# HUSRCF/JaTSR-Just-audio-transformer-super-solution

Measured on AMD Instinct MI355X. Metric: DiT latent-frames/sec (B=28,C=1024,T=512, 50-step CFG), higher is better.
Workload: dtype bf16; 1 GPU; v3mod2 DiT 50-step CFG=3.0 flow-matching sampling, hipGraph, B=28/GPU C=1024 T=512; B_per_gpu=28, global_batch=28, T=512, C=1024, euler_steps=50, weights=recipe (random-init, non-zero adaLN/final), parallelism=replicas x1, no collective in the loop, rccl_ranks=1

## Files before the change

jatsr-just-audio-transformer-super-solution_amd/csrc/elementwise.hip:

```cpp
#include "jat_kernels.h"
#include "jat_gelu.h"
#include "jat_dtype.h"
#include <cstdlib>

__device__ __forceinline__ unsigned short f2bf_e(float f) { return jat_f2op(f); }
__device__ __forceinline__ uint2 pack4_e(float a, float b, float c, float d) {
  uint2 r;
  r.x = jat_pack2(a, b);
  r.y = jat_pack2(c, d);
  return r;
}
__device__ __forceinline__ float wave_sum(float v) {
#pragma unroll
  for (int o = 32; o > 0; o >>= 1) v += __shfl_xor(v, o);
  return v;
}
__device__ __forceinline__ float silu_f(float x) { return x / (1.0f + __expf(-x)); }

__global__ void __launch_bounds__(256) norm_modulate_kernel(const float* __restrict__ x, const float* __restrict__ w,
                                                            const float* __restrict__ shift,
                                                            const float* __restrict__ scale, int64_t mod_bstride,
                                                            bf16_t* __restrict__ y, int M, int D, int ntok, int mode) {
  const int lane = threadIdx.x & 63;
  const int row = blockIdx.x * 4 + (threadIdx.x >> 6);
// ... 184 lines not shown
      const uint2 v = *(const uint2*)(tile + r * ROW + part * 8);
      *(uint2*)(A + ((int64_t)b * ntok + tok0 + r) * Ktot + (int64_t)c0 * 4 + part * 4) = v;
    }
  }
}

hipError_t launch_patchify(const float* x_t, const float* x_cond, bf16_t* A, int B, int B_src, int cond_zero_from,
                           int C_t, int C_c, int T_orig, int ntok, hipStream_t s, const int* tvalid) {
  if (C_t % 32 != 0 || C_c % 32 != 0 || B <= 0 || B_src <= 0) return hipErrorInvalidValue;
  dim3 grid((ntok + 63) / 64, (C_t + C_c) / 32, B);
  hipLaunchKernelGGL(patchify_kernel, grid, dim3(256), 0, s, x_t, x_cond, A, B_src, cond_zero_from, C_t, C_c, T_orig,
                     ntok, tvalid);
  return hipGetLastError();
}

__global__ void time_sinusoid_kernel(const float* __restrict__ t, float* __restrict__ e, int B, int D) {
  const int half = D >> 1;
  const int i = blockIdx.x * blockDim.x + threadIdx.x;
  if (i >= B * half) return;
  const int b = i / half, k = i - b * half;
  const float c = logf(10000.0f) / (float)(half - 1);
  const float f = expf((float)k * -c);
  const float a = t[b] * f;
  e[(int64_t)b * D + k] = sinf(a);
  e[(int64_t)b * D + half + k] = cosf(a);
}
hipError_t launch_time_sinusoid(const float* t, float* e, int B, int D, hipStream_t s) {
  const int n = B * (D / 2);
  hipLaunchKernelGGL(time_sinusoid_kernel, dim3((n + 255) / 256), dim3(256), 0, s, t, e, B, D);
  return hipGetLastError();
// ... 392 lines not shown
```

jatsr-just-audio-transformer-super-solution_amd/csrc/gemm.hip:

```cpp
#include "jat_kernels.h"
#include "jat_dtype.h"

#include <type_traits>

typedef jat_opx8 bf16x8;
typedef __attribute__((ext_vector_type(4))) float f32x4;
typedef __attribute__((ext_vector_type(4))) unsigned u32x4;
typedef __attribute__((address_space(3))) void* lds_ptr_t;

template <int I, int N, class F>
__device__ __forceinline__ void static_for(F&& f) {
  if constexpr (I < N) {
    f(std::integral_constant<int, I>{});
    static_for<I + 1, N>(f);
  }
}

__device__ __forceinline__ unsigned short f2bf(float f) { return jat_f2op(f); }
__device__ __forceinline__ uint2 pack4(float a, float b, float c, float d) {
  uint2 r;
  r.x = jat_pack2(a, b);
  r.y = jat_pack2(c, d);
  return r;
}
#include "jat_gelu.h"
__device__ __forceinline__ uint2 gelu_pack4(float a, float b, float c, float d) {
  f32x2 g[2] = {f32x2{a, b}, f32x2{c, d}};
  gelu_erf_n<2>(g);
  return pack4(g[0][0], g[0][1], g[1][0], g[1][1]);
}

__device__ __forceinline__ float2 rope_rot(float a, float b, float c, float s) {
  return float2{__builtin_fmaf(a, c, -(b * s)), __builtin_fmaf(b, c, a * s)};
}

template <int TM>
__device__ __forceinline__ void rows_rstd_issue(const GemmArgs& p, int row0, int lane, f32x4 (&rsv)[TM]) {
  const int lg = p.rs_np >> 3;
  const int rpi = 64 >> lg;
#pragma unroll
  for (int t = 0; t < TM; ++t) {
    const int row = min(row0 + t * rpi + (lane >> lg), p.M - 1);
    const float* ptr = p.rs_part + (int64_t)row * p.rs_np + (lane & ((1 << lg) - 1)) * 4;
    asm volatile("global_load_dwordx4 %0, %1, off" : "=v"(rsv[t]) : "v"(ptr) : "memory");
  }
}
template <int TM, int YOUNGER>
__device__ __forceinline__ void rows_rstd_reduce(const GemmArgs& p, f32x4 (&rsv)[TM], float (&sums)[TM]) {
  asm volatile("s_waitcnt vmcnt(%0)" ::"n"(YOUNGER) : "memory");
#pragma unroll
  for (int t = 0; t < TM; ++t) asm volatile("" : "+v"(rsv[t]));
  const int lpr = p.rs_np >> 2;
#pragma unroll
  for (int t = 0; t < TM; ++t) {
    float sq = (rsv[t][0] + rsv[t][1]) + (rsv[t][2] + rsv[t][3]);
    if (lpr >= 2) sq += __shfl_xor(sq, 1);
    if (lpr >= 4) sq += __shfl_xor(sq, 2);
// ... 53 lines not shown
  JAT_TL(0) JAT_TLR(5)
#else
#define JAT_TL(i)
#define JAT_TLX(i)
#define JAT_TLR(i)
#define JAT_TL_FLUSH()
#endif
  if (p.ksplit > 1) {
    const int z = blockIdx.y;
    p.A += (int64_t)z * p.K;
    p.W += (int64_t)z * p.K;
    p.out = (float*)p.out + (int64_t)z * p.split_stride;
  }
  constexpr int BM = WM * TM * 16, BN = WN * TN * 16, BK = 64;
  constexpr int NW = WM * WN;
  constexpr int A_BYTES = BM * 128, B_BYTES = BN * 128, STAGE = A_BYTES + B_BYTES;
  constexpr int PA = BM / 8, PB = BN / 8;
  constexpr int AI = (PA + NW - 1) / NW, BI = (PB + NW - 1) / NW;
  static_assert(BM % 8 == 0 && BN % 8 == 0, "tile rows must be a multiple of 8");
  extern __shared__ __attribute__((aligned(16))) char smem[];

  const int tid = threadIdx.x, lane = tid & 63;
  const int wave = __builtin_amdgcn_readfirstlane(tid >> 6);
  const int wm = wave / WN, wn = wave % WN;

  const int tiles_m = (p.M + BM - 1) / BM, tiles_n = p.N / BN;
  int id;
  {
    const int nwg = gridDim.x, bid = blockIdx.x;
    const int q = nwg >> 3, r = nwg & 7, xcd = bid & 7;
    id = (xcd < r ? xcd * (q + 1) : r * (q + 1) + (xcd - r) * q) + (bid >> 3);
  }
  constexpr int GROUP = 8;
  const int per_group = GROUP * tiles_n;
  const int first_m = (id / per_group) * GROUP;
  const int gsz = min(tiles_m - first_m, GROUP);
  const int in_g = id % per_group;
  const int m0 = (first_m + in_g % gsz) * BM;
  const int n0 = (in_g / gsz) * BN;

  const int srow = lane >> 3;
  const int schunk = (lane & 7) ^ srow;
  const bf16_t* a_src[AI];
  const bf16_t* b_src[BI];
#pragma unroll
  for (int j = 0; j < AI; ++j) {
    const int r = min(wave + j * NW, PA - 1) * 8 + srow;
    const int gm = min(m0 + r, p.M - 1);
    a_src[j] = p.A + (int64_t)gm * p.lda + schunk * 8;
  }
#pragma unroll
  for (int j = 0; j < BI; ++j) {
    const int r = min(wave + j * NW, PB - 1) * 8 + srow;
// ... 41 lines not shown
    for (int j = 0; j < TN; ++j) wf[j] = *(const bf16x8*)(sB + b_row_off + j * 2048 + coff);
  };
  auto mma = [&](const bf16x8(&af)[TM], const bf16x8(&wf)[TN]) {
#pragma unroll
    for (int i = 0; i < TM; ++i)
#pragma unroll
      for (int j = 0; j < TN; ++j)
        acc[i][j] = JAT_MFMA_16x16x32(wf[j], af[i], acc[i][j], 0, 0, 0);
  };

  float rstd_rows[TM], rstd_sums[TM];
  [[maybe_unused]] f32x4 rstd_raw[TM];
#pragma unroll
  for (int i = 0; i < TM; ++i) rstd_rows[i] = 1.0f;
  if (p.rs_part) {
    rows_rstd_issue<TM>(p, m0 + wm * TM * 16, lane, rstd_raw);
    if constexpr (PIPE != 8) rows_rstd_reduce<TM, 0>(p, rstd_raw, rstd_sums);
  }

  const int nk = p.K / BK;
  if constexpr (PIPE == 6) {
    static_assert(NW == 8 && PA % 4 == 0 && PB % 4 == 0, "PIPE 6: 8 MFMA waves + 4 DMA waves");
    constexpr int NDW = 4, AI6 = PA / NDW, BI6 = PB / NDW;
    if (wave >= NW) {
      const int dw = wave - NW;
      const bf16_t* asrc[AI6];
      const bf16_t* bsrc[BI6];
#pragma unroll
      for (int j = 0; j < AI6; ++j)
        asrc[j] = p.A + (int64_t)min(m0 + (dw + j * NDW) * 8 + srow, p.M - 1) * p.lda + schunk * 8;
#pragma unroll
// ... 55 lines not shown
      cur = cur == 2 ? 0 : cur + 1;
    }
    if (grp == 0) __builtin_amdgcn_s_barrier();
  } else if constexpr (PIPE == 8) {
    static_assert(NW == 8, "quadrant ping-pong needs two waves per SIMD in one block");
    constexpr bool SPLIT_M = TM * TN > 20;
    constexpr int TMa = SPLIT_M ? (TM + 1) / 2 : TM, TMb = TM - TMa, TNa = (TN + 1) / 2, TNb = TN - TNa;
    constexpr int PA0 = WM * TMa * 2, PA1 = WM * TMb * 2, PB0 = WN * TNa * 2, PB1 = WN * TNb * 2;
    constexpr int CA0 = (PA0 + 7) / 8, CA1 = (PA1 + 7) / 8, CB0 = (PB0 + 7) / 8, CB1 = (PB1 + 7) / 8;
    constexpr int CTILE = CA0 + CA1 + CB0 + CB1;
    const int grp = wave >> 2;
    const char* a_base = (const char*)(p.A + (int64_t)m0 * p.lda);
    const char* b_base = (const char*)(p.W + (int64_t)n0 * p.ldw);
    unsigned oa0[CA0], oa1[CA1 > 0 ? CA1 : 1], ob0[CB0], ob1[CB1];
    int la0[CA0], la1[CA1 > 0 ? CA1 : 1], lb0[CB0], lb1[CB1];
    auto piece_row = [&](int q, int per, int tiles, int first) {
      const int w = q / per, in = q - w * per;
      return w * tiles * 16 + first * 16 + in * 8;
    };
#pragma unroll
    for (int j = 0; j < CA0; ++j) {
      const int r = piece_row(min(wave + 8 * j, PA0 - 1), TMa * 2, TM, 0);
      oa0[j] = (unsigned)((min(m0 + r + srow, p.M - 1) - m0) * (int)p.lda * 2 + schunk * 16);
      la0[j] = r * 128;
    }
#pragma unroll
    for (int j = 0; j < CA1; ++j) {
      const int r = piece_row(min(wave + 8 * j, PA1 - 1), TMb * 2, TM, TMa);
      oa1[j] = (unsigned)((min(m0 + r + srow, p.M - 1) - m0) * (int)p.lda * 2 + schunk * 16);
      la1[j] = r * 128;
    }
    auto piece_row_b = [&](int q, int per, int first) {
      const int w = q / per, in = q - w * per;
      return ctile(w, first + (in >> 1)) * 16 + (in & 1) * 8;
    };
#pragma unroll
    for (int j = 0; j < CB0; ++j) {
      const int r = piece_row_b(min(wave + 8 * j, PB0 - 1), TNa * 2, 0);
      ob0[j] = (unsigned)((r + srow) * (int)p.ldw * 2 + schunk * 16);
      lb0[j] = A_BYTES + r * 128;
    }
#pragma unroll
    for (int j = 0; j < CB1; ++j) {
      const int r = piece_row_b(min(wave + 8 * j, PB1 - 1), TNb * 2, TNa);
// ... 625 lines not shown
        const int d = dt * 16 + frow, ch = kk * 4 + fg;
        const bf16x8 vf = *(const bf16x8*)(smem + SV + d * 256 + (ch >> 3) * 128 + (((ch & 7) ^ (d & 7)) << 4));
#pragma unroll
        for (int h = 0; h < G; ++h) o[h][dt] = JAT_MFMA_16x16x32(vf, pf[h][kk], o[h][dt], 0, 0, 0);
      }
    JAT_TLX(4)
    if (m0 + q < p.M) {
#pragma unroll
      for (int h = 0; h < G; ++h) {
        bf16_t* op = (bf16_t*)p.out + (int64_t)(m0 + q) * p.ldo + (hbase + h) * 64 + fg * 4;
#pragma unroll
        for (int dt = 0; dt < 4; ++dt)
          *(uint2*)(op + dt * 16) = pack4(o[h][dt][0] * inv[h], o[h][dt][1] * inv[h], o[h][dt][2] * inv[h], o[h][dt][3] * inv[h]);
      }
    }
    JAT_TL_FLUSH()
    return;
  }

#pragma unroll
  for (int i = 0; i < TM; ++i) {
    const int m = m0 + wm * TM * 16 + i * 16 + frow;
    if (m >= p.M) continue;
    int b = 0, pos = m;
    if constexpr (EPI == EPI_RESID || EPI == EPI_QKV_ROPE || EPI == EPI_UNPATCH) {
      b = m / p.ntok;
      pos = m - b * p.ntok;
    }
    const float rstd_d = rstd_rows[i];
#pragma unroll
// ... 660 lines not shown
}

template <int WM, int WN, int TM, int TN, int PIPE, int CE, int EPI>
static hipError_t launch_one(const GemmArgs& a, hipStream_t s) {
  constexpr int BM = WM * TM * 16, BN = WN * TN * 16;
  constexpr int LDS = (PIPE == 6 ? 3 : 2) * (BM + BN) * 128;
  static_assert(LDS <= 160 * 1024, "tile does not fit the 160 KiB LDS");
  static bool attr_set = false;
  auto kern = gemm_bf16_kernel<WM, WN, TM, TN, PIPE, CE, EPI>;
  if (!attr_set) {
    hipError_t e = hipFuncSetAttribute((const void*)kern, hipFuncAttributeMaxDynamicSharedMemorySize, LDS);
    if (e != hipSuccess) return e;
    attr_set = true;
  }
  if (a.N % BN != 0 || a.K % 64 != 0 || a.M <= 0) return hipErrorInvalidValue;
  const int tiles = ((a.M + BM - 1) / BM) * (a.N / BN);
  if (a.ksplit > 1 && EPI != EPI_F32) return hipErrorInvalidValue;
  hipLaunchKernelGGL(kern, dim3(tiles, a.ksplit > 1 ? a.ksplit : 1), dim3((WM * WN + (PIPE == 6 ? 4 : 0)) * 64), LDS, s, a);
  return hipGetLastError();
}

template <int WM, int WN, int TM, int TN, int PIPE, int CE = 0>
static hipError_t launch_epi(const GemmArgs& a, int epi, hipStream_t s) {
  switch (epi) {
    case EPI_F32: return launch_one<WM, WN, TM, TN, PIPE, CE, EPI_F32>(a, s);
    case EPI_BF16: return launch_one<WM, WN, TM, TN, PIPE, CE, EPI_BF16>(a, s);
    case EPI_BF16_GELU: return launch_one<WM, WN, TM, TN, PIPE, CE, EPI_BF16_GELU>(a, s);
    case EPI_RESID: return launch_one<WM, WN, TM, TN, PIPE, CE, EPI_RESID>(a, s);
    case EPI_QKV_ROPE: return launch_one<WM, WN, TM, TN, PIPE, CE, EPI_QKV_ROPE>(a, s);
    case EPI_UNPATCH: return launch_one<WM, WN, TM, TN, PIPE, CE, EPI_UNPATCH>(a, s);
  }
// ... 24 lines not shown

hipError_t launch_qkv_attn(const GemmArgs& a, hipStream_t s) {
  if (a.ntok != 128 || a.N % 448 != 0 || a.M % 128 != 0) return hipErrorInvalidValue;
  return launch_one<2, 4, 4, 7, 8, 0, EPI_QKV_ATTN>(a, s);
}
void gemm_variant_tile(int variant, int* bm, int* bn) {
  *bm = kVariantTile[variant][0];
  *bn = kVariantTile[variant][1];
}

bool gemm_variant_exists(int variant) {
  return variant >= 0 && variant < gemm_num_variants() && kVariantTile[variant][0] != 0;
}

hipError_t launch_gemm(const GemmArgs& a, int epi, int variant, hipStream_t s) {
  if (!gemm_variant_exists(variant)) return hipErrorInvalidValue;
  if (a.N % kVariantTile[variant][1] != 0) variant = (a.N % 128 == 0) ? 20 : 10;
  switch (variant) {
    case 10: return launch_epi<2, 2, 4, 2, 1>(a, epi, s);
    case 18: return launch_epi<2, 2, 4, 5, 2, 1>(a, epi, s);
    case 20: return launch_epi<2, 2, 4, 4, 2, 1>(a, epi, s);
    case 21: return launch_epi<2, 4, 8, 4, 2, 1>(a, epi, s);
    case 25: return launch_epi<4, 2, 4, 5, 6, 1>(a, epi, s);
    case 26: return launch_epi<4, 2, 4, 4, 6, 1>(a, epi, s);
    case 27: return launch_epi<2, 2, 2, 5, 2, 1>(a, epi, s);
    case 28: return launch_epi<2, 2, 2, 4, 2, 1>(a, epi, s);
    case 31: return launch_epi<2, 4, 7, 5, 8, 1>(a, epi, s);
    case 39:
      if (gemm_kpair_part_eligible(a, epi)) return launch_kpair<EPI_F32, 0, true>(a, s);
      if (gemm_kpair_eligible(a, epi))
// ... 14 lines not shown
```

jatsr-just-audio-transformer-super-solution_amd/csrc/jat_api.cpp:

```cpp
#include "../../include/jat_hip.h"

#include <hip/hip_runtime.h>

#include <cmath>
#include <cstdarg>
#include <cstdio>
#include <cstdlib>
#include <cstring>
#include <string>
#include <unordered_map>
#include <vector>

#include "jat_internal.h"
#include "jat_dtype.h"

static thread_local char g_err[512] = "";
int jat_fail(int code, const char* fmt, ...) {
  va_list ap;
  va_start(ap, fmt);
  vsnprintf(g_err, sizeof(g_err), fmt, ap);
  va_end(ap);
  return code;
}

// ... 478 lines not shown
      JCHK(gemm(m, G_FC2, w.hm, m->mlp, L.w2, m->mlp, M, D, m->mlp, EPI_F32, p, s));
      if (can_fuse && !f && next) {
        KCHK(launch_splitk_resid_norm(w.kpart, split, (int64_t)M * D, L.b2, mod_l + 5 * D, bstride, w.x, next->w, next->shift,
                                      next->scale, bstride, w.xn, M, D, ntok, m->cfg.norm_mode, s));
        if (next_done) *next_done = true;
      } else {
        KCHK(launch_splitk_resid_finish(w.kpart, split, (int64_t)M * D, L.b2, mod_l + 5 * D, bstride, ntok, w.x, M, D, s));
      }
    } else {
      JCHK(gemm(m, G_FC2, w.hm, m->mlp, L.w2, m->mlp, M, D, m->mlp, EPI_RESID, e, s));
    }
  }
  return JAT_OK;
}

static int forward_impl(const jat_model* m, const Workspace& w, const float* x_t, int B_src, const float* x_cond,
                        int cond_zero_from, const float* t, const float* mod, int64_t mod_bstride, float* x_pred,
                        int B, int T, hipStream_t s, const Fold* f = nullptr, const float* pc = nullptr) {
  const int ntok = (T + 3) / 4, M = B * ntok, D = m->D;
  if (!mod) {
    JCHK(time_path(m, w, t, B, s));
    JCHK(adaln_path(m, w.t_silu, w.mod, B, 0, m->depth, s));
    mod = w.mod;
    mod_bstride = (int64_t)m->depth * 6 * D;
  }
  if (t) HIPCHK(hipMemsetAsync(w.vt, 0, w.vt_bytes, s));
  auto patch_split = [&](int rows, int K) {
    if (!m->sw.patch_split || m->variants[G_OTHER] >= 0 || m->bott % 128 != 0) return 1;
    const int tiles = ((rows + 63) / 64) * (m->bott / 128);
    if (tiles > 128 && K < 8192) return 1;
    int split = 512 / tiles, cap = m->mlp / (2 * m->bott);
    if (cap > 4) cap = 4;
    if (split > cap) split = cap;
    while (split > 1 && ((K / 64) % split != 0 || K / split < 1024)) --split;
    return split > 1 ? split : 1;
  };
  if (pc) {
    const int Mh = M / 2, Kz = m->P * m->Cin;
    KCHK(launch_patchify(x_t, nullptr, w.a_patch, B_src, B_src, B_src, m->Cin, 0, T, ntok, s, w.tvalid));
    const int ps = patch_split(Mh, Kz);
    if (ps > 1) {
      GemmArgs e{};
      e.out = w.hm; e.ldo = m->bott; e.ntok = ntok; e.ksplit = ps; e.split_stride = (int64_t)Mh * m->bott;
      JCHK(gemm(m, G_OTHER, w.a_patch, Kz, m->pe_w1, m->Kp, Mh, m->bott, Kz, EPI_F32, e, s));
      KCHK(launch_splitk_gelu_finish((const float*)w.hm, ps, (int64_t)Mh * m->bott, m->pe_b1, pc, Mh, w.h_patch, m->bott, Mh, m->bott, s));
    } else {
      GemmArgs e{};
      e.out = w.h_patch; e.ldo = m->bott; e.bias = m->pe_b1; e.ntok = ntok; e.dual_add = pc; e.dual_rows = Mh;
      JCHK(gemm(m, G_OTHER, w.a_patch, Kz, m->pe_w1, m->Kp, Mh, m->bott, Kz, EPI_BF16_GELU, e, s));
    }
  } else {
    KCHK(launch_patchify(x_t, x_cond, w.a_patch, B, B_src, cond_zero_from, m->Cin, m->Cc, T, ntok, s, w.tvalid));
    const int ps = patch_split(M, m->Kp);
    if (ps > 1) {
// ... 11 lines not shown
    GemmArgs e{};
    e.out = w.x; e.ldo = D; e.bias = m->pe_b2; e.ntok = ntok;
    if (f) { e.fold_out = w.xn; e.fold_lo = w.xlo; e.fold_part = w.part; }
    JCHK(gemm(m, G_OTHER, w.h_patch, m->bott, m->pe_w2, m->bott, M, D, m->bott, EPI_F32, e, s));
  }
  bool xn_ready = false;
  for (int l = 0; l < m->depth; ++l) {
    const float* mod_n = mod + (int64_t)(l + 1) * 6 * D;
    const NextNorm nn = l + 1 < m->depth ? NextNorm{m->layers[l + 1].norm1, mod_n + 0 * D, mod_n + 1 * D}
                                         : NextNorm{m->final_norm, nullptr, nullptr};
    bool done = false;
    JCHK(run_block(m, w, l, B, ntok, mod + (int64_t)l * 6 * D, mod_bstride, s, f, xn_ready, &nn, &done));
    xn_ready = done;
  }
  if (!f && !xn_ready) KCHK(launch_norm_modulate(w.x, m->final_norm, nullptr, nullptr, 0, w.xn, M, D, ntok, m->cfg.norm_mode, s));
  {
    GemmArgs e{};
    e.out = x_pred; e.bias = m->bfinal; e.ntok = ntok; e.C_out = m->Cin; e.T_orig = T;
    if (f) e.rs_part = w.part;
    JCHK(gemm(m, G_OTHER, w.xn, D, f ? f->wfinal : m->wfinal, D, M, m->Fout, D, EPI_UNPATCH, e, s));
  }
  return JAT_OK;
}

static int check_ready(const jat_model* m, int B, int ntok, void* ws, size_t ws_bytes, Workspace* w) {
  if (!m) return fail(JAT_E_INVALID, "null model");
  if (!m->loaded) return fail(JAT_E_STATE, "weights not loaded");
  if (B <= 0 || ntok <= 0) return fail(JAT_E_INVALID, "B and T must be positive");
  if (ntok > MAX_LEN) return fail(JAT_E_SEQLEN, "Sequence length %d exceeds max_len %d", ntok, MAX_LEN);
  *w = carve(m, B, ntok, (char*)ws);
  if (!ws || ws_bytes < w->total)
// ... 68 lines not shown

struct jat_sampler {
  jat_model* m;
  int B, T, steps, Bf;
  float cfg_scale;
  bool use_cfg;
  std::vector<float> ts;
  char* blob = nullptr;
  float *z, *lr, *xpred, *mod_table, *ts_dev;
  std::shared_ptr<FoldTable> fold;
  bool fused_attn = false;
  float* pc = nullptr;
  int* lens_dev = nullptr;
  int* frames_dev = nullptr;
  bool folded = false;
  void* ws;
  size_t ws_bytes;
  Workspace w;
  hipStream_t cap_stream = nullptr;
  hipGraph_t graph = nullptr;
  hipGraphExec_t exec = nullptr;
};

static void linspace01(int n, std::vector<float>& out) {
  out.resize(n);
  const float step = 1.0f / (float)(n - 1);
  for (int i = 0; i < n; ++i)
    out[i] = i < n / 2 ? (float)((double)step * i) : (float)(1.0 - (double)step * (n - 1 - i));
}

static int sampler_cond_part(jat_sampler* sp, hipStream_t s) {
  if (!sp->pc) return JAT_OK;
  jat_model* m = sp->m;
  const int ntok = (sp->T + 3) / 4, Kc = m->P * m->Cc;
  KCHK(launch_patchify(sp->lr, nullptr, sp->w.a_patch, sp->B, sp->B, sp->B, m->Cc, 0, sp->T, ntok, s, sp->w.tvalid));
  GemmArgs e{};
  e.out = sp->pc; e.ldo = m->bott; e.ntok = ntok;
  return gemm(m, G_OTHER, sp->w.a_patch, Kc, m->pe_w1 + (int64_t)m->P * m->Cin, m->Kp, sp->B * ntok, m->bott, Kc, EPI_F32, e, s);
}

static int sampler_steps(jat_sampler* sp, hipStream_t s) {
  jat_model* m = sp->m;
  const int64_t n_half = (int64_t)sp->B * m->Cin * sp->T;
  const int64_t row = (int64_t)m->depth * 6 * m->D;
  for (int i = 0; i < sp->steps; ++i) {
    const float t_curr = sp->ts[i], dt = sp->ts[i + 1] - sp->ts[i];
    Fold f{};
    if (sp->folded) {
      const FoldTable& ft = *sp->fold;
      const int64_t Nqkv = m->D + 2 * m->kvD, dl = m->depth;
      if (sp->fused_attn) { f.wqkv_g = ft.qkv_g + (int64_t)i * dl * Nqkv * m->D; f.bq_g = ft.bq_g + (int64_t)i * dl * Nqkv; }
      else { f.wqkv_i = ft.qkv_i + (int64_t)i * dl * Nqkv * m->D; f.bq_i = ft.bq_i + (int64_t)i * dl * Nqkv; }
      f.w1 = ft.w1 + (int64_t)i * dl * m->mlp * m->D;
      f.bf = ft.bf + (int64_t)i * dl * m->mlp;
      f.wfinal = ft.wfinal;
    }
    JCHK(forward_impl(m, sp->w, sp->z, sp->B, sp->lr, sp->B, nullptr, sp->mod_table + i * row, 0, sp->xpred, sp->Bf,
                      sp->T, s, sp->folded ? &f : nullptr, sp->pc));
    KCHK(launch_cfg_euler(sp->xpred, sp->z, sp->cfg_scale, t_curr, dt, sp->use_cfg ? 1 : 0, n_half, s));
  }
  return JAT_OK;
}

static int fold_alloc(FoldTable& ft, void** p, size_t bytes) {
  if (hipMalloc(p, bytes) != hipSuccess) { (void)hipGetLastError(); return fail(JAT_E_HIP, "hipMalloc(%zu) for the folded weights", bytes); }
  ft.allocs.push_back(*p);
  return JAT_OK;
}
static int build_fold_table_impl(jat_model* m, FoldTable& ft, int steps, const float* mod, bool group_major, bf16_t* sh_bf16,
                                 hipStream_t s, bool need_w1, bool need_qkv);
// ... 83 lines not shown
  const int ntok = (T + 3) / 4;
  if (ntok > MAX_LEN) return fail(JAT_E_SEQLEN, "Sequence length %d exceeds max_len %d", ntok, MAX_LEN);
  HIPCHK(hipDeviceSynchronize());
  jat_sampler* sp = new jat_sampler();
  sp->m = m; sp->B = B; sp->T = T; sp->steps = steps; sp->cfg_scale = cfg_scale;
  sp->use_cfg = cfg_scale != 1.0f;
  sp->Bf = sp->use_cfg ? 2 * B : B;
  linspace01(steps + 1, sp->ts);

  const size_t lat = (size_t)B * m->Cin * T * 4;
  const size_t row = (size_t)m->depth * 6 * m->D;
  const int Bws = sp->Bf > steps ? sp->Bf : steps;
  const size_t ws_bytes = carve(m, Bws, ntok, nullptr).total;
  size_t off = 0;
  auto take = [&](size_t bytes) { size_t o = off; off += align_up(bytes, 256); return o; };
  const size_t o_z = take(lat), o_lr = take(lat), o_xp = take((size_t)sp->Bf * m->Cin * T * 4);
  const size_t o_tab = take((size_t)steps * row * 4), o_ts = take((size_t)steps * 4), o_ws = take(ws_bytes);
  const int fold_env = m->sw.fold_norm;
  {
    const int M = sp->Bf * ntok;
    auto var = [&](int site) { return m->variants[site] >= 0 ? m->variants[site] : pick_variant(M, m->D); };
    const int np = m->D / gemm_variant_wave_n(var(G_OUT));
    sp->folded = fold_env > 0 && m->cfg.norm_mode == JAT_NORM_RMS_W && m->fold_src_ok && (np == 4 || np == 8 || np == 16) &&
                 gemm_variant_coalesced(var(G_OUT)) && gemm_variant_coalesced(var(G_FC2)) && gemm_variant_coalesced(var(G_OTHER)) &&
                 gemm_variant_wave_n(var(G_OUT)) == gemm_variant_wave_n(var(G_FC2)) &&
                 gemm_variant_wave_n(var(G_OUT)) == gemm_variant_wave_n(var(G_OTHER)) &&
                 (M > kSplitMaxRows || fold_env >= 2);
    const int fuse_env = m->sw.fuse_qkv_attn;
    sp->fused_attn = fuse_env && m->Hq / m->Hkv == 5 && !m->group_copy_stale && ntok == 128 && (sp->Bf * m->Hkv >= 192 || fuse_env == 2);
  }
  const size_t o_sh = take((size_t)steps * m->D * 2);
  const size_t o_lens = take((size_t)sp->Bf * 4), o_frames = take((size_t)B * 4);
  const size_t o_pc = take((size_t)B * ntok * m->bott * 4);
  hipError_t e = hipMalloc((void**)&sp->blob, off);
  if (e != hipSuccess) { delete sp; return fail(JAT_E_HIP, "hipMalloc(%zu): %s", off, hipGetErrorString(e)); }
  sp->z = (float*)(sp->blob + o_z); sp->lr = (float*)(sp->blob + o_lr); sp->xpred = (float*)(sp->blob + o_xp);
  sp->mod_table = (float*)(sp->blob + o_tab); sp->ts_dev = (float*)(sp->blob + o_ts);
  sp->ws = sp->blob + o_ws; sp->ws_bytes = ws_bytes;
  bf16_t* sh_bf16 = (bf16_t*)(sp->blob + o_sh);
  sp->lens_dev = (int*)(sp->blob + o_lens);
  sp->frames_dev = (int*)(sp->blob + o_frames);
  if (sp->use_cfg && m->sw.split_patch) sp->pc = (float*)(sp->blob + o_pc);

  int rc = JAT_OK;
  auto bail = [&](int code) { jat_sampler_destroy(sp); return code; };
  if (hipStreamCreateWithFlags(&sp->cap_stream, hipStreamNonBlocking) != hipSuccess)
    return bail(fail(JAT_E_HIP, "hipStreamCreate failed"));
  hipStream_t s = sp->cap_stream;

  {
    Workspace wt = carve(m, steps, ntok, (char*)sp->ws);
// ... 23 lines not shown
  if (hipMemsetAsync(sp->w.vt, 0, sp->w.vt_bytes, s) != hipSuccess) return bail(fail(JAT_E_HIP, "memset vt"));
  {
    std::vector<int> full((size_t)sp->Bf, ntok), fullT((size_t)B, T);
    if (hipMemcpyAsync(sp->lens_dev, full.data(), full.size() * 4, hipMemcpyHostToDevice, s) != hipSuccess ||
        hipMemcpyAsync(sp->frames_dev, fullT.data(), fullT.size() * 4, hipMemcpyHostToDevice, s) != hipSuccess ||
        hipStreamSynchronize(s) != hipSuccess)
      return bail(fail(JAT_E_HIP, "lengths upload"));
    if (!sp->fused_attn) { sp->w.lens = sp->lens_dev; sp->w.tvalid = sp->frames_dev; }
  }

  if (hipMemsetAsync(sp->z, 0, lat, s) != hipSuccess || hipMemsetAsync(sp->lr, 0, lat, s) != hipSuccess)
    return bail(fail(JAT_E_HIP, "memset"));
  {
    const int saved = sp->steps;
    sp->steps = 1;
    if ((rc = sampler_cond_part(sp, s)) != JAT_OK) return bail(rc);
    rc = sampler_steps(sp, s);
    sp->steps = saved;
    if (rc != JAT_OK) return bail(rc);
    if (hipStreamSynchronize(s) != hipSuccess)
      return bail(fail(JAT_E_HIP, "eager warm-up step failed: %s", hipGetErrorString(hipGetLastError())));
  }
  if (hipStreamBeginCapture(s, hipStreamCaptureModeRelaxed) != hipSuccess)
    return bail(fail(JAT_E_HIP, "hipStreamBeginCapture failed"));
  rc = sampler_steps(sp, s);
  e = hipStreamEndCapture(s, &sp->graph);
  if (rc != JAT_OK) return bail(rc);
  if (e != hipSuccess) return bail(fail(JAT_E_HIP, "hipStreamEndCapture: %s", hipGetErrorString(e)));
  e = hipGraphInstantiate(&sp->exec, sp->graph, nullptr, nullptr, 0);
  if (e != hipSuccess) return bail(fail(JAT_E_HIP, "hipGraphInstantiate: %s", hipGetErrorString(e)));
  *out = sp;
// ... 26 lines not shown
  if (sp->fused_attn && !all_full)
    return fail(JAT_E_STATE, "this bucket runs the fused QKV+attention kernel (128 tokens), which has no key mask");
  hipStream_t s = (hipStream_t)stream;
  HIPCHK(hipMemcpyAsync(sp->lens_dev, tok.data(), tok.size() * 4, hipMemcpyHostToDevice, s));
  HIPCHK(hipMemcpyAsync(sp->frames_dev, frames, (size_t)sp->B * 4, hipMemcpyHostToDevice, s));
  HIPCHK(hipStreamSynchronize(s));
  return JAT_OK;
}

extern "C" int jat_sampler_run(jat_sampler* sp, const float* lr_latent, const float* z0, float* z_out,
                               int32_t use_graph, void* stream) {
  if (!sp || !lr_latent || !z0 || !z_out) return fail(JAT_E_INVALID, "null argument");
  hipStream_t s = (hipStream_t)stream;
  const size_t lat = (size_t)sp->B * sp->m->Cin * sp->T * 4;
  HIPCHK(hipMemcpyAsync(sp->lr, lr_latent, lat, hipMemcpyDeviceToDevice, s));
  HIPCHK(hipMemcpyAsync(sp->z, z0, lat, hipMemcpyDeviceToDevice, s));
  JCHK(sampler_cond_part(sp, s));
  if (use_graph) {
    HIPCHK(hipGraphLaunch(sp->exec, s));
  } else {
    JCHK(sampler_steps(sp, s));
  }
  HIPCHK(hipMemcpyAsync(z_out, sp->z, lat, hipMemcpyDeviceToDevice, s));
  return JAT_OK;
}

extern "C" int jat_cfg_euler_step(const float* x_pred_2B, float* z, float cfg_scale, float t, float dt, int32_t B,
                                  int32_t C, int32_t T, void* stream) {
  KCHK(launch_cfg_euler(x_pred_2B, z, cfg_scale, t, dt, cfg_scale != 1.0f ? 1 : 0, (int64_t)B * C * T,
                        (hipStream_t)stream));
  return JAT_OK;
}

extern "C" int jat_channel_affine(const float* in, const float* mean, const float* std, float* out, int32_t B, int32_t C,
                                  int32_t T, int32_t inverse, void* stream) {
  KCHK(launch_channel_affine(in, mean, std, out, B, C, T, inverse, (hipStream_t)stream));
  return JAT_OK;
}
// ... 140 lines not shown
```

jatsr-just-audio-transformer-super-solution_amd/csrc/jat_kernels.h:

```cpp
#pragma once
#include <hip/hip_runtime.h>
#include <stdint.h>

#include "jat_rng.h"

typedef uint16_t bf16_t;

enum GemmEpi : int {
  EPI_F32 = 0,
  EPI_BF16 = 1,
  EPI_BF16_GELU = 2,
  EPI_RESID = 3,
  EPI_QKV_ROPE = 4,
  EPI_QKV_ATTN = 6,
  EPI_UNPATCH = 5,
};

struct GemmArgs {
  const bf16_t* A;
  const bf16_t* W;
  int64_t lda, ldw;
  int M, N, K;
  void* out;
  int64_t ldo;
  const float* bias;
  const float* gate;
  int64_t gate_bstride;
  int ntok;
  bf16_t* k_out;
  bf16_t* vt_out;
// ... 2 lines not shown
  const float* rope_sin;
  const float* rope_inv_freq;
  int C_out, T_orig;
  bf16_t* fold_out;
  bf16_t* fold_lo;
  float* fold_part;
  int fold_np;
  const float* rs_part;
  int rs_np;
  float attn_scale_log2e;
  const float* dual_add;
  int dual_rows;
  unsigned long long* dbg_out;
  int ksplit;
  int64_t split_stride;
  int variant_hint;
};

hipError_t launch_gemm(const GemmArgs& a, int epi, int variant, hipStream_t s);
int gemm_num_variants();
bool gemm_variant_exists(int variant);
hipError_t launch_qkv_attn(const GemmArgs& a, hipStream_t s);
void gemm_variant_tile(int variant, int* bm, int* bn);
int gemm_variant_wave_n(int variant);
bool gemm_variant_coalesced(int variant);

struct AttnArgs {
  const bf16_t* q;
  const bf16_t* k;
  const bf16_t* vt;
// ... 24 lines not shown
hipError_t launch_splitk_resid_norm(const float* part, int nsplit, int64_t stride, const float* bias, const float* gate,
                                    int64_t gate_bstride, float* x, const float* w, const float* shift, const float* scale,
                                    int64_t mod_bstride, bf16_t* y, int M, int D, int ntok, int mode, hipStream_t s);
hipError_t launch_splitk_resid_finish(const float* part, int nsplit, int64_t stride, const float* bias, const float* gate,
                                      int64_t gate_bstride, int ntok, float* x, int M, int N, hipStream_t s);
hipError_t launch_silu_bf16(const float* in, bf16_t* out, int64_t n, hipStream_t s);
hipError_t launch_cast_bf16(const float* in, bf16_t* out, int64_t n, hipStream_t s);
hipError_t launch_cast_bf16_rope_rows(const float* in, bf16_t* out, int rows, int cols, hipStream_t s);
hipError_t launch_fold_weight(const float* in, const float* w, const float* scale, bf16_t* out, int rows, int cols, int rope,
                              hipStream_t s);
hipError_t launch_fold_scale(const float* w, const float* scale, int64_t in_stride, float* out, int64_t out_stride,
                             int rows, int cols, hipStream_t s);
hipError_t launch_gather_cast_rows(const float* in, int64_t in_stride, bf16_t* out, int rows, int cols, hipStream_t s);
hipError_t launch_cfg_euler(const float* xp, float* z, float cfg_scale, float t, float dt, int use_cfg,
                            int64_t n_per_half, hipStream_t s);
hipError_t launch_channel_affine(const float* in, const float* mean, const float* std, float* out, int B,
                                 int C, int T, int inverse, hipStream_t s);
hipError_t launch_crossfade_pair(const float* prev, int Tp, const float* cur, int Tc, int overlap,
                                 float* out, int rows, hipStream_t s);

hipError_t launch_sum_partials(const float* part, int nsplit, int64_t stride, float* out, int64_t n, hipStream_t s);
hipError_t launch_transpose_bf16(const bf16_t* in, int64_t ld_in, int M, int C, bf16_t* out, int Mpad, hipStream_t s);
hipError_t launch_rowsum_bf16(const bf16_t* x, int64_t ld, int R, int n, float* out, hipStream_t s);
bool gemm_tn_supports(int M, int N);
int gemm_tn_ksplit(int M, int N, int K);
hipError_t launch_gemm_tn(const bf16_t* dY, int64_t ldy, const bf16_t* X, int64_t ldx, float* dW, int64_t ldo, int M, int N, int K,
                          int ksplit, int64_t split_stride, const void* zeros, hipStream_t s);
int colsum_slices(int R);
hipError_t launch_colsum_bf16(const bf16_t* x, int64_t ld, int R, int C, float* part, float* out, hipStream_t s);
hipError_t launch_gelu_bf16(const bf16_t* in, bf16_t* out, int64_t n, DropSpec drop, hipStream_t s);
// ... 38 lines not shown
```

Baseline: 38160 latent-frames/s.

## Fuse CFG combine and Euler update into final projection GEMM epilogue with token-layout state

Adds an EPI_CFG_EULER GEMM epilogue. Each tile computes the matching conditional and unconditional rows, exchanges them through LDS, applies CFG and the Euler update, and writes both the new fp32 state and the bf16 patch input for the next step. The sampler state is kept in token layout for the whole loop and converted only at the start and end, so the per-step unpatchify, cfg_euler and patchify kernels and the x_pred buffer are no longer needed. In exchange the epilogue is more complex, launches a fixed tile config, and relies on layout assumptions (Fout%256, T%4) with an equivalent-precision division path.

```diff
diff --git a/jatsr-just-audio-transformer-super-solution_amd/csrc/elementwise.hip b/jatsr-just-audio-transformer-super-solution_amd/csrc/elementwise.hip
--- a/jatsr-just-audio-transformer-super-solution_amd/csrc/elementwise.hip
+++ b/jatsr-just-audio-transformer-super-solution_amd/csrc/elementwise.hip
@@ -222,6 +222,70 @@
   return hipGetLastError();
 }
 
+__global__ void __launch_bounds__(256) state_to_tokens_kernel(const float* __restrict__ z, float* __restrict__ zt,
+                                                              bf16_t* __restrict__ A, int C, int T, int ntok,
+                                                              const int* __restrict__ tvalid) {
+  constexpr int ROW = 32 * 16 + 16;
+  __shared__ __attribute__((aligned(16))) char tile[64 * ROW];
+  const int tid = threadIdx.x, tok0 = blockIdx.x * 64, c0 = blockIdx.y * 32, b = blockIdx.z;
+  const int tl = tid & 63, tok = tok0 + tl;
+  const float* src = z + ((int64_t)b * C + c0) * T;
+#pragma unroll
+  for (int j = 0; j < 8; ++j) {
+    const int ci = (tid >> 6) + 4 * j;
+    float4 v = float4{0.f, 0.f, 0.f, 0.f};
+    if (tok < ntok) v = *(const float4*)(src + (int64_t)ci * T + tok * 4);
+    *(float4*)(tile + tl * ROW + ci * 16) = v;
+  }
+  __syncthreads();
+  const int tv = tvalid ? min(tvalid[b], T) : T;
+  const int K = C * 4;
+#pragma unroll
+  for (int j = 0; j < 8; ++j) {
+    const int id = tid + 256 * j, r = id >> 5, part = id & 31;
+    if (tok0 + r < ntok) {
+      const float4 v = *(const float4*)(tile + r * ROW + part * 16);
+      const int64_t o = ((int64_t)b * ntok + tok0 + r) * K + (int64_t)(c0 + part) * 4;
+      const int t0 = (tok0 + r) * 4;
+      *(float4*)(zt + o) = v;
+      *(uint2*)(A + o) = pack4_e(t0 + 0 < tv ? v.x : 0.f, t0 + 1 < tv ? v.y : 0.f, t0 + 2 < tv ? v.z : 0.f, t0 + 3 < tv ? v.w : 0.f);
+    }
+  }
+}
+__global__ void __launch_bounds__(256) state_from_tokens_kernel(const float* __restrict__ zt, float* __restrict__ z, int C,
+                                                                int T, int ntok) {
+  constexpr int ROW = 32 * 16 + 16;
+  __shared__ __attribute__((aligned(16))) char tile[64 * ROW];
+  const int tid = threadIdx.x, tok0 = blockIdx.x * 64, c0 = blockIdx.y * 32, b = blockIdx.z;
+  const int K = C * 4;
+#pragma unroll
+  for (int j = 0; j < 8; ++j) {
+    const int id = tid + 256 * j, r = id >> 5, part = id & 31;
+    if (tok0 + r < ntok)
+      *(float4*)(tile + r * ROW + part * 16) = *(const float4*)(zt + ((int64_t)b * ntok + tok0 + r) * K + (int64_t)(c0 + part) * 4);
+  }
+  __syncthreads();
+  const int tl = tid & 63, tok = tok0 + tl;
+  float* dst = z + ((int64_t)b * C + c0) * T;
+#pragma unroll
+  for (int j = 0; j < 8; ++j) {
+    const int ci = (tid >> 6) + 4 * j;
+    if (tok < ntok) *(float4*)(dst + (int64_t)ci * T + tok * 4) = *(const float4*)(tile + tl * ROW + ci * 16);
+  }
+}
+hipError_t launch_state_to_tokens(const float* z, float* zt, bf16_t* A, int B, int C, int T, const int* tvalid, hipStream_t s) {
+  if (C % 32 != 0 || T % 4 != 0 || B <= 0 || T <= 0) return hipErrorInvalidValue;
+  const int ntok = T / 4;
+  hipLaunchKernelGGL(state_to_tokens_kernel, dim3((ntok + 63) / 64, C / 32, B), dim3(256), 0, s, z, zt, A, C, T, ntok, tvalid);
+  return hipGetLastError();
+}
+hipError_t launch_state_from_tokens(const float* zt, float* z, int B, int C, int T, hipStream_t s) {
+  if (C % 32 != 0 || T % 4 != 0 || B <= 0 || T <= 0) return hipErrorInvalidValue;
+  const int ntok = T / 4;
+  hipLaunchKernelGGL(state_from_tokens_kernel, dim3((ntok + 63) / 64, C / 32, B), dim3(256), 0, s, zt, z, C, T, ntok);
+  return hipGetLastError();
+}
+
 __global__ void time_sinusoid_kernel(const float* __restrict__ t, float* __restrict__ e, int B, int D) {
   const int half = D >> 1;
   const int i = blockIdx.x * blockDim.x + threadIdx.x;
diff --git a/jatsr-just-audio-transformer-super-solution_amd/csrc/gemm.hip b/jatsr-just-audio-transformer-super-solution_amd/csrc/gemm.hip
--- a/jatsr-just-audio-transformer-super-solution_amd/csrc/gemm.hip
+++ b/jatsr-just-audio-transformer-super-solution_amd/csrc/gemm.hip
@@ -35,12 +35,12 @@
 }
 
 template <int TM>
-__device__ __forceinline__ void rows_rstd_issue(const GemmArgs& p, int row0, int lane, f32x4 (&rsv)[TM]) {
+__device__ __forceinline__ void rows_rstd_issue(const GemmArgs& p, int row0, int row_max, int lane, f32x4 (&rsv)[TM]) {
   const int lg = p.rs_np >> 3;
   const int rpi = 64 >> lg;
 #pragma unroll
   for (int t = 0; t < TM; ++t) {
-    const int row = min(row0 + t * rpi + (lane >> lg), p.M - 1);
+    const int row = min(row0 + t * rpi + (lane >> lg), row_max);
     const float* ptr = p.rs_part + (int64_t)row * p.rs_np + (lane & ((1 << lg) - 1)) * 4;
     asm volatile("global_load_dwordx4 %0, %1, off" : "=v"(rsv[t]) : "v"(ptr) : "memory");
   }
@@ -124,6 +124,9 @@
   }
   constexpr int BM = WM * TM * 16, BN = WN * TN * 16, BK = 64;
   constexpr int NW = WM * WN;
+  constexpr bool PAIR = EPI == EPI_CFG_EULER;
+  static_assert(!PAIR || (WM == 2 && PIPE == 8), "CFG/Euler epilogue: two wave rows (cond, uncond) and the PIPE 8 A-row map");
+  constexpr int RM = PAIR ? BM / 2 : BM;
   constexpr int A_BYTES = BM * 128, B_BYTES = BN * 128, STAGE = A_BYTES + B_BYTES;
   constexpr int PA = BM / 8, PB = BN / 8;
   constexpr int AI = (PA + NW - 1) / NW, BI = (PB + NW - 1) / NW;
@@ -134,7 +137,7 @@
   const int wave = __builtin_amdgcn_readfirstlane(tid >> 6);
   const int wm = wave / WN, wn = wave % WN;
 
-  const int tiles_m = (p.M + BM - 1) / BM, tiles_n = p.N / BN;
+  const int tiles_m = (p.M + RM - 1) / RM, tiles_n = p.N / BN;
   int id;
   {
     const int nwg = gridDim.x, bid = blockIdx.x;
@@ -146,7 +149,7 @@
   const int first_m = (id / per_group) * GROUP;
   const int gsz = min(tiles_m - first_m, GROUP);
   const int in_g = id % per_group;
-  const int m0 = (first_m + in_g % gsz) * BM;
+  const int m0 = (first_m + in_g % gsz) * RM;
   const int n0 = (in_g / gsz) * BN;
 
   const int srow = lane >> 3;
@@ -218,7 +221,8 @@
 #pragma unroll
   for (int i = 0; i < TM; ++i) rstd_rows[i] = 1.0f;
   if (p.rs_part) {
-    rows_rstd_issue<TM>(p, m0 + wm * TM * 16, lane, rstd_raw);
+    if constexpr (PAIR) rows_rstd_issue<TM>(p, wm * p.M + m0, wm * p.M + p.M - 1, lane, rstd_raw);
+    else rows_rstd_issue<TM>(p, m0 + wm * TM * 16, p.M - 1, lane, rstd_raw);
     if constexpr (PIPE != 8) rows_rstd_reduce<TM, 0>(p, rstd_raw, rstd_sums);
   }
 
@@ -304,6 +308,14 @@
     const char* b_base = (const char*)(p.W + (int64_t)n0 * p.ldw);
     unsigned oa0[CA0], oa1[CA1 > 0 ? CA1 : 1], ob0[CB0], ob1[CB1];
     int la0[CA0], la1[CA1 > 0 ? CA1 : 1], lb0[CB0], lb1[CB1];
+    auto a_rel = [&](int r) {
+      if constexpr (PAIR) {
+        const int h = r >= RM;
+        return h * p.M + min(m0 + r - h * RM, p.M - 1) - m0;
+      } else {
+        return min(m0 + r, p.M - 1) - m0;
+      }
+    };
     auto piece_row = [&](int q, int per, int tiles, int first) {
       const int w = q / per, in = q - w * per;
       return w * tiles * 16 + first * 16 + in * 8;
@@ -311,13 +323,13 @@
 #pragma unroll
     for (int j = 0; j < CA0; ++j) {
       const int r = piece_row(min(wave + 8 * j, PA0 - 1), TMa * 2, TM, 0);
-      oa0[j] = (unsigned)((min(m0 + r + srow, p.M - 1) - m0) * (int)p.lda * 2 + schunk * 16);
+      oa0[j] = (unsigned)(a_rel(r + srow) * (int)p.lda * 2 + schunk * 16);
       la0[j] = r * 128;
     }
 #pragma unroll
     for (int j = 0; j < CA1; ++j) {
       const int r = piece_row(min(wave + 8 * j, PA1 - 1), TMb * 2, TM, TMa);
-      oa1[j] = (unsigned)((min(m0 + r + srow, p.M - 1) - m0) * (int)p.lda * 2 + schunk * 16);
+      oa1[j] = (unsigned)(a_rel(r + srow) * (int)p.lda * 2 + schunk * 16);
       la1[j] = r * 128;
     }
     auto piece_row_b = [&](int q, int per, int first) {
@@ -973,6 +985,79 @@
           *(uint2*)(op + dt * 16) = pack4(o[h][dt][0] * inv[h], o[h][dt][1] * inv[h], o[h][dt][2] * inv[h], o[h][dt][3] * inv[h]);
       }
     }
+    JAT_TL_FLUSH()
+    return;
+  }
+
+  if constexpr (PAIR) {
+    constexpr int HT = (TM + 1) / 2;
+    constexpr int XB = TM * TN * 1024;
+    static_assert(WN * XB <= 2 * STAGE, "exchange image does not fit the staging buffers");
+    float4 bb[TN];
+#pragma unroll
+    for (int j = 0; j < TN; ++j)
+      bb[j] = p.bias ? *(const float4*)(p.bias + nw0 + j * 16 + fg * 4) : float4{0.f, 0.f, 0.f, 0.f};
+    {
+#pragma clang fp contract(off)
+#pragma unroll
+      for (int i = 0; i < TM; ++i)
+#pragma unroll
+        for (int j = 0; j < TN; ++j) {
+          const float bj[4] = {bb[j].x, bb[j].y, bb[j].z, bb[j].w};
+#pragma unroll
+          for (int r = 0; r < 4; ++r) acc[i][j][r] = acc[i][j][r] * rstd_rows[i] + bj[r];
+        }
+    }
+    f32x4 zr[HT][TN];
+    auto zrow = [&](int i) { return m0 + i * 16 + frow; };
+    auto load_z = [&](auto I0, auto NI) {
+#pragma unroll
+      for (int k = 0; k < decltype(NI)::value; ++k) {
+        const int m = zrow(decltype(I0)::value + k);
+#pragma unroll
+        for (int j = 0; j < TN; ++j)
+          zr[k][j] = m < p.M ? *(const f32x4*)((const float*)p.out + (int64_t)m * p.ldo + nw0 + j * 16 + fg * 4) : f32x4{0.f, 0.f, 0.f, 0.f};
+      }
+    };
+    if (wm == 0) load_z(std::integral_constant<int, 0>{}, std::integral_constant<int, HT>{});
+    else load_z(std::integral_constant<int, HT>{}, std::integral_constant<int, TM - HT>{});
+    char* xbuf = smem + wn * XB + lane * 16;
+    __syncthreads();
+#pragma unroll
+    for (int i = 0; i < TM; ++i)
+      if ((wm == 0) == (i >= HT))
+#pragma unroll
+        for (int j = 0; j < TN; ++j) *(f32x4*)(xbuf + (i * TN + j) * 1024) = acc[i][j];
+    __syncthreads();
+    const float cs = p.cfg_scale, denom = p.euler_denom, dt = p.euler_dt;
+    auto finish = [&](auto I0, auto NI) {
+#pragma unroll
+      for (int k = 0; k < decltype(NI)::value; ++k) {
+        const int i = decltype(I0)::value + k;
+        const int m = zrow(i);
+        if (m >= p.M) continue;
+        const int b = m / p.ntok, pos = m - b * p.ntok;
+        const int tv = p.tvalid ? p.tvalid[b] : 0x7fffffff;
+#pragma unroll
+        for (int j = 0; j < TN; ++j) {
+          const f32x4 other = *(const f32x4*)(xbuf + (i * TN + j) * 1024);
+          const f32x4 c = wm == 0 ? acc[i][j] : other, u = wm == 0 ? other : acc[i][j];
+          f32x4 zn;
+#pragma unroll
+          for (int r = 0; r < 4; ++r) {
+            const float x = __builtin_fmaf(cs, c[r] - u[r], u[r]);
+            zn[r] = p.euler_direct ? x : __builtin_fmaf(__fdiv_rn(x - zr[k][j][r], denom), dt, zr[k][j][r]);
+          }
+          const int n = nw0 + j * 16 + fg * 4;
+          *(f32x4*)((float*)p.out + (int64_t)m * p.ldo + n) = zn;
+          const int t0 = pos * 4;
+          *(uint2*)(p.a_next + (int64_t)m * p.ldo + n) = pack4(t0 + 0 < tv ? zn[0] : 0.f, t0 + 1 < tv ? zn[1] : 0.f,
+                                                               t0 + 2 < tv ? zn[2] : 0.f, t0 + 3 < tv ? zn[3] : 0.f);
+        }
+      }
+    };
+    if (wm == 0) finish(std::integral_constant<int, 0>{}, std::integral_constant<int, HT>{});
+    else finish(std::integral_constant<int, HT>{}, std::integral_constant<int, TM - HT>{});
     JAT_TL_FLUSH()
     return;
   }
@@ -1663,7 +1748,8 @@
     attr_set = true;
   }
   if (a.N % BN != 0 || a.K % 64 != 0 || a.M <= 0) return hipErrorInvalidValue;
-  const int tiles = ((a.M + BM - 1) / BM) * (a.N / BN);
+  constexpr int RM = EPI == EPI_CFG_EULER ? BM / 2 : BM;
+  const int tiles = ((a.M + RM - 1) / RM) * (a.N / BN);
   if (a.ksplit > 1 && EPI != EPI_F32) return hipErrorInvalidValue;
   hipLaunchKernelGGL(kern, dim3(tiles, a.ksplit > 1 ? a.ksplit : 1), dim3((WM * WN + (PIPE == 6 ? 4 : 0)) * 64), LDS, s, a);
   return hipGetLastError();
@@ -1718,6 +1804,11 @@
 }
 
 hipError_t launch_gemm(const GemmArgs& a, int epi, int variant, hipStream_t s) {
+  if (epi == EPI_CFG_EULER) {
+    if (a.ksplit > 1 || !a.a_next || a.ldo % 4 != 0 || a.ntok <= 0 || 2 * (int64_t)a.M * a.lda * 2 >= (1ll << 31))
+      return hipErrorInvalidValue;
+    return launch_one<2, 4, 7, 4, 8, 1, EPI_CFG_EULER>(a, s);
+  }
   if (!gemm_variant_exists(variant)) return hipErrorInvalidValue;
   if (a.N % kVariantTile[variant][1] != 0) variant = (a.N % 128 == 0) ? 20 : 10;
   switch (variant) {
diff --git a/jatsr-just-audio-transformer-super-solution_amd/csrc/jat_api.cpp b/jatsr-just-audio-transformer-super-solution_amd/csrc/jat_api.cpp
--- a/jatsr-just-audio-transformer-super-solution_amd/csrc/jat_api.cpp
+++ b/jatsr-just-audio-transformer-super-solution_amd/csrc/jat_api.cpp
@@ -516,9 +516,13 @@
   return JAT_OK;
 }
 
+struct EulerStep { float* z; float cfg_scale, denom, dt; int direct; };
+
 static int forward_impl(const jat_model* m, const Workspace& w, const float* x_t, int B_src, const float* x_cond,
                         int cond_zero_from, const float* t, const float* mod, int64_t mod_bstride, float* x_pred,
-                        int B, int T, hipStream_t s, const Fold* f = nullptr, const float* pc = nullptr) {
+                        int B, int T, hipStream_t s, const Fold* f = nullptr, const float* pc = nullptr,
+                        const EulerStep* eu = nullptr) {
+  if (eu && !pc) return fail(JAT_E_INVALID, "the fused CFG/Euler step needs the split patch embed");
   const int ntok = (T + 3) / 4, M = B * ntok, D = m->D;
   if (!mod) {
     JCHK(time_path(m, w, t, B, s));
@@ -539,7 +543,7 @@
   };
   if (pc) {
     const int Mh = M / 2, Kz = m->P * m->Cin;
-    KCHK(launch_patchify(x_t, nullptr, w.a_patch, B_src, B_src, B_src, m->Cin, 0, T, ntok, s, w.tvalid));
+    if (!eu) KCHK(launch_patchify(x_t, nullptr, w.a_patch, B_src, B_src, B_src, m->Cin, 0, T, ntok, s, w.tvalid));
     const int ps = patch_split(Mh, Kz);
     if (ps > 1) {
       GemmArgs e{};
@@ -581,7 +585,13 @@
     xn_ready = done;
   }
   if (!f && !xn_ready) KCHK(launch_norm_modulate(w.x, m->final_norm, nullptr, nullptr, 0, w.xn, M, D, ntok, m->cfg.norm_mode, s));
-  {
+  if (eu) {
+    GemmArgs e{};
+    e.out = eu->z; e.ldo = m->Fout; e.bias = m->bfinal; e.ntok = ntok; e.a_next = w.a_patch; e.tvalid = w.tvalid;
+    e.cfg_scale = eu->cfg_scale; e.euler_denom = eu->denom; e.euler_dt = eu->dt; e.euler_direct = eu->direct;
+    if (f) e.rs_part = w.part;
+    JCHK(gemm(m, G_OTHER, w.xn, D, f ? f->wfinal : m->wfinal, D, M / 2, m->Fout, D, EPI_CFG_EULER, e, s));
+  } else {
     GemmArgs e{};
     e.out = x_pred; e.bias = m->bfinal; e.ntok = ntok; e.C_out = m->Cin; e.T_orig = T;
     if (f) e.rs_part = w.part;
@@ -680,6 +690,7 @@
   int* lens_dev = nullptr;
   int* frames_dev = nullptr;
   bool folded = false;
+  bool tok_state = false;
   void* ws;
   size_t ws_bytes;
   Workspace w;
@@ -703,6 +714,13 @@
   GemmArgs e{};
   e.out = sp->pc; e.ldo = m->bott; e.ntok = ntok;
   return gemm(m, G_OTHER, sp->w.a_patch, Kc, m->pe_w1 + (int64_t)m->P * m->Cin, m->Kp, sp->B * ntok, m->bott, Kc, EPI_F32, e, s);
+}
+
+static int sampler_begin(jat_sampler* sp, const float* z0, hipStream_t s) {
+  JCHK(sampler_cond_part(sp, s));
+  if (sp->tok_state) KCHK(launch_state_to_tokens(z0, sp->z, sp->w.a_patch, sp->B, sp->m->Cin, sp->T, sp->w.tvalid, s));
+  else if (z0 != sp->z) HIPCHK(hipMemcpyAsync(sp->z, z0, (size_t)sp->B * sp->m->Cin * sp->T * 4, hipMemcpyDeviceToDevice, s));
+  return JAT_OK;
 }
 
 static int sampler_steps(jat_sampler* sp, hipStream_t s) {
@@ -720,6 +738,12 @@
       f.w1 = ft.w1 + (int64_t)i * dl * m->mlp * m->D;
       f.bf = ft.bf + (int64_t)i * dl * m->mlp;
       f.wfinal = ft.wfinal;
+    }
+    if (sp->tok_state) {
+      const EulerStep eu{sp->z, sp->cfg_scale, 1.0f - t_curr + 1e-5f, dt, !(t_curr < 0.999f)};
+      JCHK(forward_impl(m, sp->w, sp->z, sp->B, sp->lr, sp->B, nullptr, sp->mod_table + i * row, 0, nullptr, sp->Bf, sp->T, s,
+                        sp->folded ? &f : nullptr, sp->pc, &eu));
+      continue;
     }
     JCHK(forward_impl(m, sp->w, sp->z, sp->B, sp->lr, sp->B, nullptr, sp->mod_table + i * row, 0, sp->xpred, sp->Bf,
                       sp->T, s, sp->folded ? &f : nullptr, sp->pc));
@@ -833,7 +857,8 @@
   const size_t ws_bytes = carve(m, Bws, ntok, nullptr).total;
   size_t off = 0;
   auto take = [&](size_t bytes) { size_t o = off; off += align_up(bytes, 256); return o; };
-  const size_t o_z = take(lat), o_lr = take(lat), o_xp = take((size_t)sp->Bf * m->Cin * T * 4);
+  sp->tok_state = sp->use_cfg && m->sw.split_patch && T % 4 == 0 && m->Fout % 256 == 0;
+  const size_t o_z = take(lat), o_lr = take(lat), o_xp = take(sp->tok_state ? 0 : (size_t)sp->Bf * m->Cin * T * 4);
   const size_t o_tab = take((size_t)steps * row * 4), o_ts = take((size_t)steps * 4), o_ws = take(ws_bytes);
   const int fold_env = m->sw.fold_norm;
   {
@@ -853,7 +878,7 @@
   const size_t o_pc = take((size_t)B * ntok * m->bott * 4);
   hipError_t e = hipMalloc((void**)&sp->blob, off);
   if (e != hipSuccess) { delete sp; return fail(JAT_E_HIP, "hipMalloc(%zu): %s", off, hipGetErrorString(e)); }
-  sp->z = (float*)(sp->blob + o_z); sp->lr = (float*)(sp->blob + o_lr); sp->xpred = (float*)(sp->blob + o_xp);
+  sp->z = (float*)(sp->blob + o_z); sp->lr = (float*)(sp->blob + o_lr); sp->xpred = sp->tok_state ? nullptr : (float*)(sp->blob + o_xp);
   sp->mod_table = (float*)(sp->blob + o_tab); sp->ts_dev = (float*)(sp->blob + o_ts);
   sp->ws = sp->blob + o_ws; sp->ws_bytes = ws_bytes;
   bf16_t* sh_bf16 = (bf16_t*)(sp->blob + o_sh);
@@ -907,7 +932,7 @@
   {
     const int saved = sp->steps;
     sp->steps = 1;
-    if ((rc = sampler_cond_part(sp, s)) != JAT_OK) return bail(rc);
+    if ((rc = sampler_begin(sp, sp->lr, s)) != JAT_OK) return bail(rc);
     rc = sampler_steps(sp, s);
     sp->steps = saved;
     if (rc != JAT_OK) return bail(rc);
@@ -964,14 +989,14 @@
   hipStream_t s = (hipStream_t)stream;
   const size_t lat = (size_t)sp->B * sp->m->Cin * sp->T * 4;
   HIPCHK(hipMemcpyAsync(sp->lr, lr_latent, lat, hipMemcpyDeviceToDevice, s));
-  HIPCHK(hipMemcpyAsync(sp->z, z0, lat, hipMemcpyDeviceToDevice, s));
-  JCHK(sampler_cond_part(sp, s));
+  JCHK(sampler_begin(sp, z0, s));
   if (use_graph) {
     HIPCHK(hipGraphLaunch(sp->exec, s));
   } else {
     JCHK(sampler_steps(sp, s));
   }
-  HIPCHK(hipMemcpyAsync(z_out, sp->z, lat, hipMemcpyDeviceToDevice, s));
+  if (sp->tok_state) KCHK(launch_state_from_tokens(sp->z, z_out, sp->B, sp->m->Cin, sp->T, s));
+  else HIPCHK(hipMemcpyAsync(z_out, sp->z, lat, hipMemcpyDeviceToDevice, s));
   return JAT_OK;
 }
 
diff --git a/jatsr-just-audio-transformer-super-solution_amd/csrc/jat_kernels.h b/jatsr-just-audio-transformer-super-solution_amd/csrc/jat_kernels.h
--- a/jatsr-just-audio-transformer-super-solution_amd/csrc/jat_kernels.h
+++ b/jatsr-just-audio-transformer-super-solution_amd/csrc/jat_kernels.h
@@ -14,6 +14,7 @@
   EPI_QKV_ROPE = 4,
   EPI_QKV_ATTN = 6,
   EPI_UNPATCH = 5,
+  EPI_CFG_EULER = 7,
 };
 
 struct GemmArgs {
@@ -46,6 +47,10 @@
   unsigned long long* dbg_out;
   int ksplit;
   int64_t split_stride;
+  float cfg_scale, euler_denom, euler_dt;
+  int euler_direct;
+  bf16_t* a_next;
+  const int* tvalid;
   int variant_hint;
 };
 
@@ -100,6 +105,8 @@
 hipError_t launch_gather_cast_rows(const float* in, int64_t in_stride, bf16_t* out, int rows, int cols, hipStream_t s);
 hipError_t launch_cfg_euler(const float* xp, float* z, float cfg_scale, float t, float dt, int use_cfg,
                             int64_t n_per_half, hipStream_t s);
+hipError_t launch_state_to_tokens(const float* z, float* zt, bf16_t* A, int B, int C, int T, const int* tvalid, hipStream_t s);
+hipError_t launch_state_from_tokens(const float* zt, float* z, int B, int C, int T, hipStream_t s);
 hipError_t launch_channel_affine(const float* in, const float* mean, const float* std, float* out, int B,
                                  int C, int T, int inverse, hipStream_t s);
 hipError_t launch_crossfade_pair(const float* prev, int Tp, const float* cur, int Tc, int overlap,
```

Result: faster. 38620 latent-frames/s (median of 6 runs) (+1.2%).
